# sflorescu/BWA-MEM_GPU

Measured on AMD Instinct MI355X. Metric: Mreads/s (150 bp single-end vs hg38-scale index; seed-and-extend hot path), higher is better.
Workload: dtype u16

## Files before the change

### bwa-mem_gpu_amd/bwamem_hip/lib.py

```python
from __future__ import annotations

import ctypes as C
import os

import numpy as np

_PKG = os.path.dirname(os.path.dirname(os.path.abspath(__file__)))
_u8p, _u32p, _u64p, _i32p = (C.POINTER(t) for t in (C.c_uint8, C.c_uint32, C.c_uint64, C.c_int32))


class HipLibraryMissing(RuntimeError):
    pass


def lib_path() -> str:
    return os.environ.get("BMH_LIB") or os.path.join(_PKG, "libbwamem_hip.so")


EXPORTED_SYMBOLS = [
    "bmh_last_error", "bmh_device_count", "bmh_set_device", "bmh_index_upload", "bmh_index_from_device",
    "bmh_index_free", "bmh_index_probe", "bmh_index_replicate", "bmh_rccl_where", "bmh_rccl_unique_id", "bmh_rccl_comm_init_rank", "bmh_rccl_comm_destroy", "bmh_index_broadcast_rccl", "bmh_index_replicate_all", "bmh_shard_range", "bmh_index_densify_sa", "bmh_index_build", "bmh_seed_ws_create", "bmh_seed_ws_free", "bmh_seed_batch", "bmh_seed_last_timing", "bmh_reseed_opt_default", "bmh_seed_batch_reseed", "bmh_aligner_set_reseed",
    "bmh_host_pin", "bmh_host_unpin", "bmh_extend_batch", "bmh_extend_batch_long", "bmh_extend_last_ms", "bmh_extend_last_unsupported", "bmh_extend_last_class_sizes", "bmh_extend_set_packed", "bmh_tune_set", "bmh_wtrace_start", "bmh_wtrace_stop", "bmh_wtrace_kept", "bmh_extend_release", "bmh_finalize_release", "bmh_matesw_release", "bmh_calib_gather", "bmh_calib_valu", "bmh_calib_valu_placed", "bmh_calib_last_clock",
    "bmh_jobs_frac_rep", "bmh_post_opt_default", "bmh_finalize_regs", "bmh_finalize_regs_device", "bmh_finalize_regs_device_last_ms", "bmh_sam_need_cigar", "bmh_format_sam", "bmh_free",
    "bmh_pe_opt_default", "bmh_finalize_pairs", "bmh_finalize_pairs_dev", "bmh_dedup_regs_device", "bmh_finalize_pairs_deduped", "bmh_rescue_check_counts", "bmh_sam_need_cigar_pe", "bmh_format_sam_pe",
    "bmh_chain_opt_default", "bmh_chain_last_timing", "bmh_build_jobs", "bmh_jobs_free", "bmh_jobs_sizes", "bmh_jobs_arrays", "bmh_merge_regs",
    "bmh_chain_ws_create", "bmh_chain_ws_free", "bmh_chain_set_contigs", "bmh_chain_set_alt", "bmh_effective_cpus", "bmh_aligner_create", "bmh_aligner_free", "bmh_aligner_run", "bmh_aligner_run_fasta", "bmh_chain_set_materialize", "bmh_chain_batch",
    "bmh_chain_extend", "bmh_chain_merge", "bmh_chain_extend_merge", "bmh_chain_extend_merge_timing", "bmh_cigar_batch", "bmh_cigar_release",
    "bmh_sam_select_work", "bmh_sam_select_device", "bmh_cigar_pack_work", "bmh_cigar_pack_sizes", "bmh_cigar_pack", "bmh_sam_text_work", "bmh_sam_text_sizes", "bmh_sam_text_write", "bmh_sam_text_check",
    "bwt_destroy_gpu", "bwt_restore_sa_gpu", "bwt_restore_bwt_gpu", "gpu_cpy_wrapper",
    "pre_calc_seed_intervals_wrapper", "free_gpuseed_data", "seed_gpu", "seed_gpu_last_n_reads",
    "bmh_reads_load_fasta", "bmh_reads_free", "bmh_fasta_scan",
    "bmh_reads_load", "bmh_reads_scan", "bmh_format_sam_ex", "bmh_format_sam_pe_ex", "bmh_aligner_run_file",
    "bmh_chain_ws_set_max_qlen", "bmh_aligner_set_max_qlen", "bmh_aligner_host_tail_batches",
    "bmh_index_fasta", "bmh_fasta_pack", "bmh_fasta_packed_free",
    "bmh_reads_load_files", "bmh_aligner_run_files",
    "bmh_bgzf_scan", "bmh_inflate_members_device", "bmh_inflate_members_host", "bmh_inflate_status_name", "bmh_bgzf_inflate",
# ... 460 lines not shown
    p = lib_path()
    if not os.path.exists(p):
        raise HipLibraryMissing(f"{p} not found: build it with `make -C bwa-mem_gpu_amd/csrc` "
                                "(or __graft_entry__.build()); there is no CPU fallback")
    L = C.CDLL(p)
    L.bmh_last_error.restype = C.c_char_p
    L.bmh_device_count.restype = C.c_int
    L.bmh_set_device.argtypes = [C.c_int]
    L.bmh_index_upload.restype = C.c_void_p
    L.bmh_index_upload.argtypes = [C.c_uint64, _u64p, C.c_uint64, _u32p, C.c_uint64, C.c_int, _u32p, C.c_uint64,
                                   _u32p, _u8p, C.c_uint64]
    L.bmh_index_from_device.restype = C.c_void_p
    L.bmh_index_from_device.argtypes = [C.c_uint64, _u64p, C.c_uint64, C.c_void_p, C.c_uint64, C.c_int, C.c_void_p,
                                        C.c_uint64, C.c_void_p, C.c_void_p, C.c_uint64]
    L.bmh_index_free.argtypes = [C.c_void_p]
    L.bmh_tune_set.restype = C.c_int
    L.bmh_wtrace_start.restype = C.c_int
    L.bmh_wtrace_start.argtypes = [C.c_uint32]
    L.bmh_wtrace_stop.restype = C.c_int64
    L.bmh_wtrace_stop.argtypes = [C.c_void_p, C.c_uint32]
    L.bmh_wtrace_kept.restype = C.c_uint32
    L.bmh_tune_set.argtypes = [C.c_char_p, C.c_int, C.c_int]
    L.bmh_rccl_where.restype = C.c_char_p
    L.bmh_rccl_unique_id.restype = C.c_int
    L.bmh_rccl_unique_id.argtypes = [C.c_void_p]
    L.bmh_rccl_comm_init_rank.restype = C.c_int
    L.bmh_rccl_comm_init_rank.argtypes = [C.POINTER(C.c_void_p), C.c_int, C.c_void_p, C.c_int]
    L.bmh_rccl_comm_destroy.argtypes = [C.c_void_p]
    L.bmh_index_broadcast_rccl.restype = C.c_int
    L.bmh_index_broadcast_rccl.argtypes = [C.c_void_p, C.c_int, C.c_void_p, C.POINTER(C.c_void_p), C.c_void_p]
# ... 187 lines not shown
            raise RuntimeError(f"bmh_index_densify_sa rc={rc}: " + _err(L))

    def probe(self, rows, what: str) -> np.ndarray:
        import torch
        L = load_library()
        r = torch.from_numpy(np.ascontiguousarray(rows, dtype=np.uint64).view(np.int64)).cuda()
        code = {"occ4": 0, "lf": 1, "sa": 2}[what]
        out = torch.empty(r.numel() * (4 if code == 0 else 1), dtype=torch.int64, device="cuda")
        rc = L.bmh_index_probe(self.handle, r.data_ptr(), r.numel(), code, out.data_ptr(), torch.cuda.current_stream().cuda_stream)
        if rc != 0:
            raise RuntimeError(f"bmh_index_probe rc={rc}: " + _err(L))
        torch.cuda.synchronize()
        o = out.cpu().numpy().view(np.uint64)
        return o.reshape(-1, 4) if code == 0 else o

    def free(self):
        if self.handle:
            load_library().bmh_index_free(self.handle)
            self.handle = None


class SeedWorkspace:
    def __init__(self, max_reads: int, max_bases: int, max_cands: int = 0, max_occ: int = 0):
        L = load_library()
        self.handle = L.bmh_seed_ws_create(max_reads, max_bases, max_cands, max_occ)
        if not self.handle:
            raise RuntimeError("bmh_seed_ws_create: " + _err(L))

    def seed_batch(self, index: Index, reads_t, offs_t, lens_t, min_seed_len: int = 19, stream: int = 0, reseed: "ReseedOpt | None" = None) -> SeedsT:
        L = load_library()
# ... 498 lines not shown
```

### bwa-mem_gpu_amd/csrc/bmh_internal.h

```cpp
#pragma once
#include "../../include/bwamem_hip.h"
#include "fmd_dev.h"

struct bmh_index {
	fmd_dev_t dev;
	bool owns;
	bool owns_sa;
	bool owns_blocks;
	uint64_t n_words;
};

struct bmh_ext_desc_t {
	const uint8_t *reads;
	const uint8_t *pac; long long l_pac;
	const uint32_t *jq_src;
	const uint32_t *job_side;
	uint32_t max_qlen;
	const int64_t *jt0;
	uint32_t long_cap;
};
int bmh_extend_batch_desc(const bmh_ext_desc_t *desc, const uint32_t *d_qlen, const uint32_t *d_tlen, const uint32_t *d_h0, uint32_t n,
                          const bmh_ext_params_t *p, int32_t *d_out, int32_t *d_raw, void *stream);
int bmh_extend_reserve(void *stream, uint64_t n);

#ifdef __cplusplus
// ... 97 lines not shown
```

### bwa-mem_gpu_amd/csrc/c_api.hip

```cpp
#include <hip/hip_runtime.h>
#include <stdarg.h>
#include <stdio.h>
#include <stdlib.h>
#include <string.h>
#include <map>
#include <mutex>
#include <string>
#include <vector>
#include "bmh_internal.h"

static thread_local char g_err[512] = "";

static std::mutex g_tune_mu;
static std::map<std::string, int> g_tune_set;
int bmh_tune(const char *name, int dflt)
{
	{
		std::lock_guard<std::mutex> lk(g_tune_mu);
		auto it = g_tune_set.find(name);
		if (it != g_tune_set.end()) return it->second;
	}
	const std::string env = std::string("BMH_") + name;
	const char *e = getenv(env.c_str());
	return e && *e ? atoi(e) : dflt;
// ... 146 lines not shown
	          hipMalloc((void **)&d_bits, bits_words * 4) == hipSuccess;
	if (ok && pac) ok = hipMalloc((void **)&d_pac, (size_t)(l_pac / 4 + 1) + 16) == hipSuccess && hipMemset(d_pac, 0, (size_t)(l_pac / 4 + 1) + 16) == hipSuccess;
	if (ok) ok = hipMemset(d_bwt, 0, bwt_bytes) == hipSuccess;
	if (ok) ok = hipMemcpy(d_bwt, bwt_words, (size_t)n_words * 4 < bwt_bytes ? (size_t)n_words * 4 : bwt_bytes, hipMemcpyHostToDevice) == hipSuccess;
	if (ok) ok = hipMemcpy(d_sa, sa, n_sa * 4, hipMemcpyHostToDevice) == hipSuccess;
	if (ok) ok = hipMemcpy(d_bits, sa_bits, bits_words * 4, hipMemcpyHostToDevice) == hipSuccess;
	if (ok && pac) ok = hipMemcpy(d_pac, pac, (size_t)(l_pac / 4 + 1), hipMemcpyHostToDevice) == hipSuccess;
	if (ok) ok = native_blocks(d_bwt, d_bwt, seq_len);
	if (!ok) {
		bmh_set_error("bmh_index_upload: %s", hipGetErrorString(hipGetLastError()));
		if (d_bwt) (void)hipFree(d_bwt); if (d_sa) (void)hipFree(d_sa); if (d_bits) (void)hipFree(d_bits); if (d_pac) (void)hipFree(d_pac);
		free(ix);
		return nullptr;
	}
	ix->dev.blocks = (const uint4 *)d_bwt; ix->dev.sa = d_sa; ix->dev.sa_bits = d_bits; ix->dev.pac = d_pac;
	return ix;
}

extern "C" bmh_index_t *bmh_index_from_device(uint64_t primary, const uint64_t L2[5], uint64_t seq_len, const uint32_t *d_bwt_words,
                                              uint64_t n_words, int sa_intv, const uint32_t *d_sa, uint64_t n_sa,
                                              const uint32_t *d_sa_bits, const uint8_t *d_pac, uint64_t l_pac)
{
	if (!L2 || !d_bwt_words || !d_sa || !d_sa_bits) { bmh_set_error("bmh_index_from_device: null argument"); return nullptr; }
	if (check_geometry(seq_len, L2, n_words, sa_intv, n_sa) != BMH_OK) return nullptr;
	if (((uintptr_t)d_bwt_words & 31) != 0) { bmh_set_error("bmh_index_from_device: bwt words must be 32-byte aligned"); return nullptr; }
	if (n_words < (((seq_len + 63) / 64) + 1) * 8) { bmh_set_error("bmh_index_from_device: buffer must be padded to %llu words", (unsigned long long)((((seq_len + 63) / 64) + 1) * 8)); return nullptr; }
	const size_t bwt_bytes = ((size_t)((seq_len + 63) / 64) + 1) * 32;
	void *d_native = nullptr;
	if (hipMalloc(&d_native, bwt_bytes) != hipSuccess || !native_blocks(d_bwt_words, d_native, seq_len)) {
		bmh_set_error("bmh_index_from_device: native blocks: %s", hipGetErrorString(hipGetLastError()));
		if (d_native) (void)hipFree(d_native);
		return nullptr;
	}
	bmh_index *ix = (bmh_index *)calloc(1, sizeof(bmh_index));
	ix->owns = false; ix->owns_blocks = true; ix->n_words = n_words;
	fill_dev(ix, primary, L2, seq_len, sa_intv, n_sa, d_pac ? l_pac : 0);
	ix->dev.blocks = (const uint4 *)d_native; ix->dev.sa = d_sa; ix->dev.sa_bits = d_sa_bits; ix->dev.pac = d_pac;
	return ix;
}

extern "C" int bmh_index_replicate(const bmh_index_t *src, int src_device, int dst_device, bmh_index_t **out)
{
	if (!src || !out) { bmh_set_error("bmh_index_replicate: null argument"); return BMH_EINVAL; }
	*out = nullptr;
	int prev = 0;
	if (hipGetDevice(&prev) != hipSuccess) { bmh_set_error("bmh_index_replicate: no HIP device"); return BMH_ENODEV; }
	const fmd_dev_t &f = src->dev;
	const size_t bwt_bytes = ((size_t)((f.seq_len + 63) / 64) + 1) * 32, sa_bytes = (size_t)f.n_sa * 4, bits_bytes = (size_t)(f.n_sa / 32 + 1) * 4;
	const size_t pac_bytes = f.pac ? (size_t)(f.l_pac / 4 + 1) + 16 : 0;
	bmh_index *ix = (bmh_index *)calloc(1, sizeof(bmh_index));
	*ix = *src; ix->owns = true; ix->owns_sa = false; ix->owns_blocks = false;
	void *d_bwt = nullptr, *d_sa = nullptr, *d_bits = nullptr, *d_pac = nullptr;
// ... 2 lines not shown
	if (ok && pac_bytes) ok = hipMalloc(&d_pac, pac_bytes) == hipSuccess && hipMemset(d_pac, 0, pac_bytes) == hipSuccess;
	auto cp = [&](void *dst, const void *s_, size_t n) {
		return src_device == dst_device ? hipMemcpy(dst, s_, n, hipMemcpyDeviceToDevice) == hipSuccess : hipMemcpyPeer(dst, dst_device, s_, src_device, n) == hipSuccess;
	};
	ok = ok && cp(d_bwt, f.blocks, bwt_bytes) && cp(d_sa, f.sa, sa_bytes) && cp(d_bits, f.sa_bits, bits_bytes);
	if (ok && pac_bytes) ok = cp(d_pac, f.pac, (size_t)(f.l_pac / 4 + 1));
	ok = ok && hipDeviceSynchronize() == hipSuccess;
	if (!ok) {
		bmh_set_error("bmh_index_replicate (device %d -> %d): %s", src_device, dst_device, hipGetErrorString(hipGetLastError()));
		void *ps[] = {d_bwt, d_sa, d_bits, d_pac};
		for (void *p : ps) if (p) (void)hipFree(p);
		free(ix); (void)hipSetDevice(prev);
		return BMH_ENOMEM;
	}
	ix->dev.blocks = (const uint4 *)d_bwt; ix->dev.sa = (const uint32_t *)d_sa; ix->dev.sa_bits = (const uint32_t *)d_bits; ix->dev.pac = (const uint8_t *)d_pac;
	(void)hipSetDevice(prev);
	*out = ix;
	return BMH_OK;
}

extern "C" void bmh_shard_range(uint64_t n, int rank, int world, uint32_t multiple, uint64_t *lo, uint64_t *hi)
{
	if (multiple < 1) multiple = 1;
	if (world < 1) world = 1;
	const uint64_t units = n / multiple;
	uint64_t a = units * (uint64_t)rank / (uint64_t)world * multiple, b = units * (uint64_t)(rank + 1) / (uint64_t)world * multiple;
	if (rank == world - 1) b = n;
	if (lo) *lo = a;
	if (hi) *hi = b;
}
// ... 27 lines not shown
	sa_densify_kernel<<<(unsigned)(nb < (1u << 22) ? nb : (1u << 22)), 256>>>(ix->dev, new_shift, n_new, d_sa, d_bits);
	hipError_t e = hipGetLastError();
	if (e == hipSuccess) e = hipDeviceSynchronize();
	if (e != hipSuccess) { bmh_set_error("bmh_index_densify_sa: %s", hipGetErrorString(e)); (void)hipFree(d_sa); (void)hipFree(d_bits); return BMH_ENODEV; }
	if (ix->owns || ix->owns_sa) { (void)hipFree((void *)ix->dev.sa); (void)hipFree((void *)ix->dev.sa_bits); }
	ix->dev.sa = d_sa; ix->dev.sa_bits = d_bits; ix->dev.n_sa = n_new; ix->dev.sa_shift = new_shift; ix->owns_sa = true;
	return BMH_OK;
}

extern "C" void bmh_index_free(bmh_index_t *ix)
{
	if (!ix) return;
	if (ix->owns || ix->owns_blocks) (void)hipFree((void *)ix->dev.blocks);
	if (ix->owns && ix->dev.pac) (void)hipFree((void *)ix->dev.pac);
	if (ix->owns || ix->owns_sa) { (void)hipFree((void *)ix->dev.sa); (void)hipFree((void *)ix->dev.sa_bits); }
	free(ix);
}

__global__ void __launch_bounds__(256) index_probe_kernel(fmd_dev_t f, const uint64_t *__restrict__ rows, uint64_t n, int what, uint64_t *__restrict__ out)
{
	const uint64_t t = (uint64_t)blockIdx.x * blockDim.x + threadIdx.x;
	if (t >= n) return;
	const uint64_t k = rows[t];
	if (what == 0) {
		uint64_t c4[4];
		fmd_occ4(f, k, c4);
		for (int c = 0; c < 4; ++c) out[4 * t + c] = fmd_occ1(f, k, c) == c4[c] ? c4[c] : ~0ull;
	} else if (what == 1) out[t] = fmd_inv_psi(f, k);
	else out[t] = fmd_sa(f, k);
}
// ... 12 lines not shown
```

### bwa-mem_gpu_amd/csrc/fmd_dev.h

```cpp
#pragma once
#include <hip/hip_runtime.h>
#include <stdint.h>

struct fmd_dev_t {
	uint64_t primary;
	uint64_t L2[5];
	uint64_t seq_len;
	const uint4 *blocks;
	const uint32_t *sa;
	const uint32_t *sa_bits;
	uint64_t n_sa;
	int sa_shift;
	const uint8_t *pac;
	uint64_t l_pac;
	int wave_prio;
};

__device__ __forceinline__ void fmd_wave_prio(const int p)
{
	if (p == 1) __builtin_amdgcn_s_setprio(1);
	else if (p == 2) __builtin_amdgcn_s_setprio(2);
	else if (p >= 3) __builtin_amdgcn_s_setprio(3);
}

struct blk_t { uint4 occ; uint64_t lo, hi; };

__device__ __forceinline__ uint32_t sel4(int c, uint32_t v0, uint32_t v1, uint32_t v2, uint32_t v3)
{
	const bool b0 = c & 1, b1 = c & 2;
	const uint32_t lo = b0 ? v1 : v0, hi = b0 ? v3 : v2;
	return b1 ? hi : lo;
// ... 209 lines not shown
```

### bwa-mem_gpu_amd/csrc/rccl_bcast.hip

```cpp
#include <dlfcn.h>
#include <hip/hip_runtime.h>
#include <rccl/rccl.h>
#include <stdio.h>
#include <stdlib.h>
#include <string.h>
#include <mutex>
#include <vector>
#include "bmh_internal.h"

namespace {
struct rccl_api_t {
	ncclResult_t (*GetUniqueId)(ncclUniqueId *);
	ncclResult_t (*CommInitRank)(ncclComm_t *, int, ncclUniqueId, int);
	ncclResult_t (*CommInitAll)(ncclComm_t *, int, const int *);
	ncclResult_t (*CommDestroy)(ncclComm_t);
	ncclResult_t (*CommCount)(const ncclComm_t, int *);
	ncclResult_t (*CommUserRank)(const ncclComm_t, int *);
	ncclResult_t (*Broadcast)(const void *, void *, size_t, ncclDataType_t, int, ncclComm_t, hipStream_t);
	ncclResult_t (*AllReduce)(const void *, void *, size_t, ncclDataType_t, ncclRedOp_t, ncclComm_t, hipStream_t);
	ncclResult_t (*GroupStart)();
	ncclResult_t (*GroupEnd)();
	const char *(*GetErrorString)(ncclResult_t);
	const char *where;
	bool ok;
// ... 167 lines not shown
			if (!ab.bytes[k]) continue;
			const void *sendp = is_root ? s[k] : nullptr;
			void *recvp = recv ? d[k] : (void *)s[k];
			rc = bcast_bytes(R, is_root ? sendp : recvp, recvp, k == 3 ? (size_t)(f.l_pac / 4 + 1) : ab.bytes[k], root, comm, st);
		}
		const ncclResult_t g1 = R->GroupEnd();
		if (rc == BMH_OK && g1 != ncclSuccess) { bmh_set_error("ncclGroupEnd: %s", R->GetErrorString(g1)); rc = BMH_ENODEV; }
	}
	if (rc == BMH_OK && hipStreamSynchronize(st) != hipSuccess) { bmh_set_error("bmh_index_broadcast_rccl: %s", hipGetErrorString(hipGetLastError())); rc = BMH_ENODEV; }
	if (rc != BMH_OK) { for (int k = 0; k < 4; ++k) if (d[k]) (void)hipFree(d[k]); return rc; }
	if (recv) {
		bmh_index *ix = (bmh_index *)calloc(1, sizeof(bmh_index));
		ix->dev = f; ix->owns = true; ix->n_words = h.n_words;
		ix->dev.blocks = (const uint4 *)d[0]; ix->dev.sa = (const uint32_t *)d[1]; ix->dev.sa_bits = (const uint32_t *)d[2]; ix->dev.pac = (const uint8_t *)d[3];
		if (!h.has_pac) ix->dev.l_pac = 0;
		*out = ix;
	}
	return BMH_OK;
}

extern "C" int bmh_index_replicate_all(const bmh_index_t *src, int src_device, const int *devices, int n, bmh_index_t **out, int *used_rccl)
{
	if (!src || !devices || !out || n < 1) { bmh_set_error("bmh_index_replicate_all: bad argument"); return BMH_EINVAL; }
	if (used_rccl) *used_rccl = 0;
	int prev = 0;
	HCK(hipGetDevice(&prev));
	std::vector<int> devs{src_device};
	for (int k = 0; k < n; ++k) { bool seen = false; for (int d : devs) seen = seen || d == devices[k]; if (!seen) devs.push_back(devices[k]); }
	std::vector<bmh_index_t *> per_dev(devs.size(), nullptr);
	per_dev[0] = (bmh_index_t *)src;
// ... 23 lines not shown
					for (int i = 0; i < nd && rc == BMH_OK; ++i) {
						(void)hipSetDevice(devs[i]);
						rc = bcast_bytes(R, i == 0 ? s[k] : d[i][k], i == 0 ? (void *)s[k] : d[i][k], nbytes, 0, comms[i], st[i]);
					}
				}
				const ncclResult_t g1 = R->GroupEnd();
				if (rc == BMH_OK && g1 != ncclSuccess) { bmh_set_error("ncclGroupEnd: %s", R->GetErrorString(g1)); rc = BMH_ENODEV; }
				for (int i = 0; i < nd; ++i) { (void)hipSetDevice(devs[i]); if (hipStreamSynchronize(st[i]) != hipSuccess && rc == BMH_OK) { bmh_set_error("bmh_index_replicate_all: %s", hipGetErrorString(hipGetLastError())); rc = BMH_ENODEV; } }
			}
			for (int i = 0; i < nd; ++i) { (void)hipSetDevice(devs[i]); if (st[i]) (void)hipStreamDestroy(st[i]); (void)R->CommDestroy(comms[i]); }
			if (rc == BMH_OK) {
				for (int i = 1; i < nd; ++i) {
					bmh_index *ix = (bmh_index *)calloc(1, sizeof(bmh_index));
					*ix = *src; ix->owns = true; ix->owns_sa = false; ix->owns_blocks = false;
					ix->dev.blocks = (const uint4 *)d[i][0]; ix->dev.sa = (const uint32_t *)d[i][1]; ix->dev.sa_bits = (const uint32_t *)d[i][2]; ix->dev.pac = (const uint8_t *)d[i][3];
					per_dev[i] = ix;
				}
				done = true;
				if (used_rccl) *used_rccl = 1;
			} else {
				for (int i = 1; i < nd; ++i) { (void)hipSetDevice(devs[i]); for (void *p : d[i]) if (p) (void)hipFree(p); }
			}
		}
	}
	if (!done) {
		for (int i = 1; i < nd; ++i)
			if (bmh_index_replicate(src, src_device, devs[i], &per_dev[i]) != BMH_OK) {
				for (int q = 1; q < i; ++q) { (void)hipSetDevice(devs[q]); bmh_index_free(per_dev[q]); }
				(void)hipSetDevice(prev);
				return BMH_ENOMEM;
// ... 8 lines not shown
```

### bwa-mem_gpu_amd/csrc/seed_kernels.hip

```cpp
#include <cstring>
#include <string>
#include <vector>
#include <hip/hip_runtime.h>
#include <rocprim/rocprim.hpp>
#include <stdint.h>
#include <stdio.h>
#include <stdlib.h>
#include "bmh_internal.h"
#include "wtrace.h"
#include "fmd_dev.h"
#include "seed_dev.h"


__device__ __forceinline__ int ascii_code(uint8_t ch)
{
	ch &= 0xDF;
	return ch == 'A' ? 0 : ch == 'C' ? 1 : ch == 'G' ? 2 : ch == 'T' ? 3 : 4;
}

#define PACK_READS_PER_BLOCK 64
__global__ void __launch_bounds__(256) pack_reads_kernel(const uint8_t *__restrict__ ascii, const uint32_t *__restrict__ offs,
                                                         const uint32_t *__restrict__ lens, uint32_t n_reads, uint32_t n_grp,
                                                         uint32_t lds_bytes, uint32_t *__restrict__ pk, uint32_t *__restrict__ nm)
{
// ... 73 lines not shown
                                                           unsigned long long *counter, uint64_t cap, uint32_t *__restrict__ n_cand,
                                                           unsigned long long *__restrict__ fst, const uint32_t *__restrict__ deal, uint32_t *__restrict__ iters_out)
{
	wtrace_scope_t wt_(WT_FORWARD);
	fmd_wave_prio(f.wave_prio);
	uint32_t r = blockIdx.x * blockDim.x + threadIdx.x;
	bool live = r < rv.n_reads;
	if (deal && live) r = deal[r];
	int len = live ? (int)lens[r] : 0;
	int i = 0, x = 0;
	uint32_t j = 0;
	uint64_t k = 0, l = 0, s = 0;
	enum { ST_START, ST_EXT, ST_DONE, ST_TAIL, ST_UNIQ };
	uint64_t tp = 0;
	int st = live && len > 0 ? ST_START : ST_DONE;
	cand_cursor_t cc = {0, 0};
	unsigned it_wave = 0, it_mine = 0;
	while (__any(st != ST_DONE)) {
		++it_wave; it_mine += st != ST_DONE ? 1u : 0u;
		bool want = false;
		cand_t c = {r, 0, 0, 0};
		uint64_t ck = 0;
		if (st == ST_START) {
			int b = read_base(rv, r, i);
			++i;
			if (b < 4) {
				x = i - 1;
				k = fmd_L2(f, b) + 1; s = fmd_L2(f, b + 1) - fmd_L2(f, b); l = fmd_L2(f, 3 - b) + 1;
				if (i == len) {
					want = i >= min_seed_len;
					c.xe = ((uint32_t)x << 16) | (uint32_t)i; c.j = j; c.s = (uint32_t)s; ck = k;
					st = ST_DONE;
				} else st = ST_EXT;
			} else if (i == len) st = ST_DONE;
		} else if (st == ST_EXT) {
			int b = read_base(rv, r, i);
			if (b < 4) {
				int cb = 3 - b;
				uint64_t ak[4], al[4], as[4];
				fmd_forward_ext(f, k, l, s, ak, al, as);
				const uint64_t ns = cb == 0 ? as[0] : cb == 1 ? as[1] : cb == 2 ? as[2] : as[3];
				const uint64_t nk = cb == 0 ? ak[0] : cb == 1 ? ak[1] : cb == 2 ? ak[2] : ak[3];
				const uint64_t nl = cb == 0 ? al[0] : cb == 1 ? al[1] : cb == 2 ? al[2] : al[3];
				if (ns != s) {
					want = i >= min_seed_len;
					c.xe = ((uint32_t)x << 16) | (uint32_t)i; c.j = j; c.s = (uint32_t)s; ck = k;
				}
				if (ns == 0) st = ST_START;
				else {
					k = nk; l = nl; s = ns; ++i;
					if (i == len) {
						st = ST_TAIL;
					} else if (s == 1 && f.pac) {
						tp = fmd_sa(f, k) + (uint64_t)(i - x);
						st = ST_UNIQ;
					}
				}
			} else {
				want = i >= min_seed_len;
				c.xe = ((uint32_t)x << 16) | (uint32_t)i; c.j = j; c.s = (uint32_t)s; ck = k;
				st = ST_START;
			}
		} else if (st == ST_TAIL) {
			want = i >= min_seed_len;
			c.xe = ((uint32_t)x << 16) | (uint32_t)i; c.j = j; c.s = (uint32_t)s; ck = k;
			st = ST_DONE;
		} else if (st == ST_UNIQ) {
			bool stop = false;
			for (int rep = 0; rep < FWD_UNIQ_WORDS && !stop && i < len; ++rep) {
				const int w16 = i & 15;
				const uint32_t rw = rv.pk[(size_t)(i >> 4) * rv.n_reads + r] >> (2 * w16);
				const uint32_t rm = rv.nm[(size_t)(i >> 5) * rv.n_reads + r] >> (i & 31);
				int n_av = min(16 - w16, len - i);
				const uint64_t room = tp < f.seq_len ? f.seq_len - tp : 0;
				n_av = (uint64_t)n_av < room ? n_av : (int)room;
				const uint32_t diff = rw ^ fmd_text16(f, tp);
				const uint32_t dp = (diff | (diff >> 1)) & 0x55555555u;
				const int fd = dp ? (__ffs((int)dp) - 1) >> 1 : 16;
				const int fn = (rm & 0xFFFFu) ? __ffs((int)(rm & 0xFFFFu)) - 1 : 16;
				const int m = min(min(fd, fn), n_av);
				stop = m < n_av || n_av == 0;
				i += m; tp += (uint64_t)m;
			}
			if (stop) {
				want = i >= min_seed_len;
				c.xe = ((uint32_t)x << 16) | (uint32_t)i; c.j = j; c.s = 1u; ck = k;
				st = ST_START;
			} else if (i == len) st = ST_TAIL;
		}
		if (want) ++j;
		cand_append(want, c, ck, out_a, out_k, counter, cap, cc);
	}
	cand_fill_invalid(cc, out_a, cap);
	if (live) n_cand[r] = j;
	if (iters_out && live) iters_out[r] = it_mine;
	if (fst) {
		if (live) { atomicAdd(fst + 1, (unsigned long long)it_mine); atomicAdd(fst + 8 + (it_mine / 8u < 31u ? it_mine / 8u : 31u), 1ull); }
		if ((threadIdx.x & 63) == 0) { atomicAdd(fst, (unsigned long long)it_wave); atomicAdd(fst + 2, 1ull); atomicMax(fst + 3, (unsigned long long)it_wave); atomicAdd(fst + 40 + (it_wave / 8u < 23u ? it_wave / 8u : 23u), 1ull); }
	}
}
// ... 76 lines not shown
			act = ok && i >= 0;
			if (act && (i & 15) == 15) {
				rw = rv.pk[(size_t)(i >> 4) * rv.n_reads + c.read];
				if ((i & 31) == 31) rm = rv.nm[(size_t)(i >> 5) * rv.n_reads + c.read];
			}
		}
		const unsigned long long am = __ballot(act) & above;
		const int nxt = am ? __builtin_ctzll(am) : lane;
		const uint32_t nsize = __shfl(size, nxt);
		if (act && am && nsize == size) { act = false; dropped = true; }
	}
	if (stats) {
		if (live && !RESUME) atomicAdd(stats + 8 + (st_mine < 39u ? st_mine : 39u), 1ull);
		atomicAdd(stats + 1, (unsigned long long)st_steps); atomicAdd(stats + 4, (unsigned long long)st_uniq); atomicAdd(stats + 5, (unsigned long long)st_u0); atomicAdd(stats + 6, (unsigned long long)st_x0); { const bool nowalk = !__any(live && !st_x0); if (!RESUME && lane == 0 && nowalk) atomicAdd(stats + 7, 1ull); }
		if (lane == 0) { atomicAdd(stats, (unsigned long long)st_iter); atomicAdd(stats + 2, 1ull); atomicMax(stats + 3, (unsigned long long)st_iter); }
	}
	const unsigned long long sm = __ballot(act);
	if (sm) {
		const int first = (int)__builtin_ctzll(sm);
		uint32_t base = 0;
		if (lane == first) base = atomicAdd(out_count, (uint32_t)__builtin_popcountll(sm));
		base = __shfl(base, first);
		if (act) {
			bwd_state_t s; s.lo = lo; s.hi = hi; s.read = c.read; s.t = t_out; s.x = (uint16_t)x; s.end = (uint16_t)end; s.i = (uint16_t)i; s.beg = (uint16_t)beg;
			out_state[base + (uint32_t)__builtin_popcountll(sm & ((1ull << lane) - 1ull))] = s;
		}
	}
	if (live && !act) {
		res_t o;
		o.read = c.read; o.be = ((uint32_t)beg << 16) | (uint32_t)end;
// ... 603 lines not shown
		HIPCK(rocprim::exclusive_scan(w->scan_tmp, tb, w->n_cand, w->cand_base, 0u, (size_t)n_reads + 1, rocprim::plus<uint32_t>(), st));
	}
	unsigned long long n_list = 0;
	uint32_t n_cands32 = 0;
	HIPCK(hipMemcpyAsync(&n_list, w->counter, 8, hipMemcpyDeviceToHost, st));
	HIPCK(hipMemcpyAsync(&n_cands32, w->cand_base + n_reads, 4, hipMemcpyDeviceToHost, st));
	HIPCK(hipStreamSynchronize(st));
	const unsigned long long n_cands = n_cands32;
	out->n_cands = n_cands;
	if (n_list > w->max_cands) { bmh_set_error("bmh_seed_batch: %llu candidate slots > capacity %llu", n_list, (unsigned long long)w->max_cands); return BMH_ECAPACITY; }
	if (n_list)
		cand_scatter_kernel<<<nblk(n_list, 256), 256, 0, st>>>(w->cand_a, n_list, w->cand_base, w->svals);
	{
		static const bool want_stats = getenv("BMH_SEED_STATS") != nullptr;
		unsigned long long *d_st = want_stats ? (unsigned long long *)w->counter + 8 : nullptr;
		if (want_stats) HIPCK(hipMemsetAsync(d_st, 0, 64 + 40 * 8, st));
		if (n_cands) {
			const std::vector<int> phases = [] {
				std::vector<int> v; const char *e = getenv("BMH_SEED_BWD_PHASES"); std::string t = e ? e : "";
				for (size_t p = 0; p < t.size();) { size_t q = t.find(',', p); if (q == std::string::npos) q = t.size(); const int k = atoi(t.substr(p, q - p).c_str()); if (k > 0) v.push_back(k); p = q + 1; }
				return v; }();
			const int np = (int)(phases.size() < 7 ? phases.size() : 7);
			const unsigned nb = nblk(n_cands, 256);
			const uint32_t sub_cap = ((nb + BWD_NSUB - 1) / BWD_NSUB) * 256u;
			if (np && bwd_state_reserve(w, (uint64_t)sub_cap * BWD_NSUB) != BMH_OK) return BMH_ENOMEM;
			uint32_t *cnt = w->bwd_cnt;
			if (np) HIPCK(hipMemsetAsync(cnt, 0, 4 * (size_t)np * BWD_NSUB, st));
			const int big = 0x7FFFFFFF;
			smem_backward_kernel<false><<<nb, 256, lds_pad, st>>>(f, rv, n_cands, min_seed_len, w->cand_a, w->cand_k, w->svals, w->res_a, w->res_k, d_st,
			                                                nullptr, nullptr, np ? w->bwd_state[0] : nullptr, np ? cnt : nullptr, sub_cap, np ? phases[0] : big);
			for (int ph = 1; ph <= np; ++ph)
				smem_backward_kernel<true><<<(sub_cap / 256u) * BWD_NSUB, 256, 0, st>>>(f, rv, n_cands, min_seed_len, w->cand_a, w->cand_k, w->svals, w->res_a, w->res_k, d_st,
				                                                                       w->bwd_state[(ph - 1) & 1], cnt + (size_t)(ph - 1) * BWD_NSUB, ph < np ? w->bwd_state[ph & 1] : nullptr,
				                                                                       ph < np ? cnt + (size_t)ph * BWD_NSUB : nullptr, sub_cap, ph < np ? phases[ph] : big);
		}
		if (want_stats) {
			unsigned long long h[48];
			HIPCK(hipStreamSynchronize(st));
			HIPCK(hipMemcpy(h, d_st, 64 + 40 * 8, hipMemcpyDeviceToHost));
			fprintf(stderr, "[backward] rank steps per candidate (0, 1, .. 38, 39+):");
			for (int q = 0; q < 40; ++q) fprintf(stderr, " %llu", h[8 + q]);
			fprintf(stderr, "\n");
			fprintf(stderr, "[backward] lane-steps on a one-row interval %llu (%.1f%%), candidates that start on one %llu (%.1f%%)\n", h[4], 100.0 * h[4] / (h[1] ? h[1] : 1), h[5], 100.0 * h[5] / (n_cands ? n_cands : 1));
			fprintf(stderr, "[backward] candidates of a pass that starts at read position 0 (no walk) %llu (%.1f%%); waves made of such only %llu\n", h[6], 100.0 * h[6] / (n_cands ? n_cands : 1), h[7]);
			fprintf(stderr, "[backward] candidates %llu, waves %llu (all phases), wave-iterations %llu (%.1f per wave, max %llu), lane-steps %llu (%.1f per candidate): lane utilisation %.1f%%\n",
			        (unsigned long long)n_cands, h[2], h[0], (double)h[0] / (h[2] ? h[2] : 1), h[3], h[1], (double)h[1] / (n_cands ? n_cands : 1), 100.0 * h[1] / (64.0 * (h[0] ? h[0] : 1)));
		}
	}
	HIPCK(hipEventRecord(w->ev[3], st));
	smem_filter_kernel<<<nblk(n_cands + 1, 256), 256, 0, st>>>(w->res_a, n_cands, w->occ);
	{
		size_t tb = w->scan_tmp_bytes;
		occ_keep_in fin; fin.occ = w->occ;
		HIPCK(rocprim::exclusive_scan(w->scan_tmp, tb, rocprim::make_transform_iterator(rocprim::counting_iterator<uint64_t>(0), fin), w->occ_off, (uint64_t)0,
		                              (size_t)n_cands + 1, rocprim::plus<uint64_t>(), st));
	}
	uint64_t tot[2] = {0, 0};
	HIPCK(hipMemcpyAsync(&tot[0], w->occ_off + n_cands, 8, hipMemcpyDeviceToHost, st));
	HIPCK(hipStreamSynchronize(st));
	tot[1] = tot[0] >> OCC_OFF_SHIFT; tot[0] &= OCC_OFF_MASK;
	if (n_cands >> 28) { bmh_set_error("bmh_seed_batch: more than 2^28 candidates in one batch"); return BMH_ECAPACITY; }
// ... 82 lines not shown
```

### include/bwamem_hip.h

```cpp
#ifndef BWAMEM_HIP_H
#define BWAMEM_HIP_H
#include <stddef.h>
#include <stdint.h>

#ifdef __cplusplus
extern "C" {
#endif

#define BMH_OK          0
#define BMH_ENODEV     -1
#define BMH_EINVAL     -2
#define BMH_ECAPACITY  -3
#define BMH_ENOMEM     -4

const char *bmh_last_error(void);
int bmh_device_count(void);
int bmh_set_device(int dev);


typedef struct bmh_index bmh_index_t;

bmh_index_t *bmh_index_upload(uint64_t primary, const uint64_t L2[5], uint64_t seq_len,
                              const uint32_t *bwt_words, uint64_t n_words, int sa_intv,
                              const uint32_t *sa, uint64_t n_sa, const uint32_t *sa_bits,
                              const uint8_t *pac, uint64_t l_pac);
bmh_index_t *bmh_index_from_device(uint64_t primary, const uint64_t L2[5], uint64_t seq_len,
                                   const uint32_t *d_bwt_words, uint64_t n_words, int sa_intv,
                                   const uint32_t *d_sa, uint64_t n_sa, const uint32_t *d_sa_bits,
                                   const uint8_t *d_pac, uint64_t l_pac);
void bmh_index_free(bmh_index_t *idx);
int bmh_index_probe(const bmh_index_t *idx, const uint64_t *d_rows, uint64_t n, int what, uint64_t *d_out, void *stream);

int bmh_index_replicate(const bmh_index_t *src, int src_device, int dst_device, bmh_index_t **out);

const char *bmh_rccl_where(void);
int bmh_rccl_unique_id(void *id128);
int bmh_rccl_comm_init_rank(void **comm, int nranks, const void *id128, int rank);
void bmh_rccl_comm_destroy(void *comm);
int bmh_index_broadcast_rccl(void *comm, int root, const bmh_index_t *src, bmh_index_t **out, void *stream);
int bmh_index_replicate_all(const bmh_index_t *src, int src_device, const int *devices, int n, bmh_index_t **out, int *used_rccl);
void bmh_shard_range(uint64_t n, int rank, int world, uint32_t multiple, uint64_t *lo, uint64_t *hi);

int bmh_index_densify_sa(bmh_index_t *idx, int new_intv);

#define BMH_BUILD_VERIFY 1
// ... 338 lines not shown
```

Before: 41.20.

## Add k-mer presence bitmap to prune seed candidates that cannot occur

```diff
diff --git a/bwa-mem_gpu_amd/bwamem_hip/lib.py b/bwa-mem_gpu_amd/bwamem_hip/lib.py
--- a/bwa-mem_gpu_amd/bwamem_hip/lib.py
+++ b/bwa-mem_gpu_amd/bwamem_hip/lib.py
@@ -19,7 +19,7 @@
 
 EXPORTED_SYMBOLS = [
     "bmh_last_error", "bmh_device_count", "bmh_set_device", "bmh_index_upload", "bmh_index_from_device",
-    "bmh_index_free", "bmh_index_probe", "bmh_index_replicate", "bmh_rccl_where", "bmh_rccl_unique_id", "bmh_rccl_comm_init_rank", "bmh_rccl_comm_destroy", "bmh_index_broadcast_rccl", "bmh_index_replicate_all", "bmh_shard_range", "bmh_index_densify_sa", "bmh_index_build", "bmh_seed_ws_create", "bmh_seed_ws_free", "bmh_seed_batch", "bmh_seed_last_timing", "bmh_reseed_opt_default", "bmh_seed_batch_reseed", "bmh_aligner_set_reseed",
+    "bmh_index_free", "bmh_index_kbits_info", "bmh_index_probe", "bmh_index_replicate", "bmh_rccl_where", "bmh_rccl_unique_id", "bmh_rccl_comm_init_rank", "bmh_rccl_comm_destroy", "bmh_index_broadcast_rccl", "bmh_index_replicate_all", "bmh_shard_range", "bmh_index_densify_sa", "bmh_index_build", "bmh_seed_ws_create", "bmh_seed_ws_free", "bmh_seed_batch", "bmh_seed_last_timing", "bmh_reseed_opt_default", "bmh_seed_batch_reseed", "bmh_aligner_set_reseed",
     "bmh_host_pin", "bmh_host_unpin", "bmh_extend_batch", "bmh_extend_batch_long", "bmh_extend_last_ms", "bmh_extend_last_unsupported", "bmh_extend_last_class_sizes", "bmh_extend_set_packed", "bmh_tune_set", "bmh_wtrace_start", "bmh_wtrace_stop", "bmh_wtrace_kept", "bmh_extend_release", "bmh_finalize_release", "bmh_matesw_release", "bmh_calib_gather", "bmh_calib_valu", "bmh_calib_valu_placed", "bmh_calib_last_clock",
     "bmh_jobs_frac_rep", "bmh_post_opt_default", "bmh_finalize_regs", "bmh_finalize_regs_device", "bmh_finalize_regs_device_last_ms", "bmh_sam_need_cigar", "bmh_format_sam", "bmh_free",
     "bmh_pe_opt_default", "bmh_finalize_pairs", "bmh_finalize_pairs_dev", "bmh_dedup_regs_device", "bmh_finalize_pairs_deduped", "bmh_rescue_check_counts", "bmh_sam_need_cigar_pe", "bmh_format_sam_pe",
@@ -510,6 +510,8 @@
     L.bmh_index_from_device.argtypes = [C.c_uint64, _u64p, C.c_uint64, C.c_void_p, C.c_uint64, C.c_int, C.c_void_p,
                                         C.c_uint64, C.c_void_p, C.c_void_p, C.c_uint64]
     L.bmh_index_free.argtypes = [C.c_void_p]
+    L.bmh_index_kbits_info.restype = C.c_int
+    L.bmh_index_kbits_info.argtypes = [C.c_void_p, C.POINTER(C.c_int), C.POINTER(C.c_void_p), _u64p]
     L.bmh_tune_set.restype = C.c_int
     L.bmh_wtrace_start.restype = C.c_int
     L.bmh_wtrace_start.argtypes = [C.c_uint32]
@@ -727,6 +729,23 @@
         o = out.cpu().numpy().view(np.uint64)
         return o.reshape(-1, 4) if code == 0 else o
 
+    def kbits_info(self) -> tuple:
+        L = load_library()
+        k, p, n = C.c_int(0), C.c_void_p(None), C.c_uint64(0)
+        rc = L.bmh_index_kbits_info(self.handle, C.byref(k), C.byref(p), C.byref(n))
+        if rc != 0:
+            raise RuntimeError(f"bmh_index_kbits_info rc={rc}: " + _err(L))
+        return int(k.value), int(p.value or 0), int(n.value)
+
+    def kbits_to_host(self) -> np.ndarray:
+        import torch
+        _, p, n = self.kbits_info()
+        if not n:
+            return np.zeros(0, np.uint32)
+        buf = torch.empty(n, dtype=torch.int32, device="cuda")
+        _memcpy_d2d(buf.data_ptr(), p, n * 4)
+        return buf.cpu().numpy().view(np.uint32)
+
     def free(self):
         if self.handle:
             load_library().bmh_index_free(self.handle)
diff --git a/bwa-mem_gpu_amd/csrc/bmh_internal.h b/bwa-mem_gpu_amd/csrc/bmh_internal.h
--- a/bwa-mem_gpu_amd/csrc/bmh_internal.h
+++ b/bwa-mem_gpu_amd/csrc/bmh_internal.h
@@ -9,6 +9,8 @@
 	bool owns_blocks;
 	uint64_t n_words;
 };
+void bmh_kbits_attach(bmh_index *ix);
+void bmh_kbits_free(bmh_index *ix);
 
 struct bmh_ext_desc_t {
 	const uint8_t *reads;
diff --git a/bwa-mem_gpu_amd/csrc/c_api.hip b/bwa-mem_gpu_amd/csrc/c_api.hip
--- a/bwa-mem_gpu_amd/csrc/c_api.hip
+++ b/bwa-mem_gpu_amd/csrc/c_api.hip
@@ -184,6 +184,7 @@
 		return nullptr;
 	}
 	ix->dev.blocks = (const uint4 *)d_bwt; ix->dev.sa = d_sa; ix->dev.sa_bits = d_bits; ix->dev.pac = d_pac;
+	bmh_kbits_attach(ix);
 	return ix;
 }
 
@@ -206,6 +207,7 @@
 	ix->owns = false; ix->owns_blocks = true; ix->n_words = n_words;
 	fill_dev(ix, primary, L2, seq_len, sa_intv, n_sa, d_pac ? l_pac : 0);
 	ix->dev.blocks = (const uint4 *)d_native; ix->dev.sa = d_sa; ix->dev.sa_bits = d_sa_bits; ix->dev.pac = d_pac;
+	bmh_kbits_attach(ix);
 	return ix;
 }
 
@@ -238,6 +240,7 @@
 		return BMH_ENOMEM;
 	}
 	ix->dev.blocks = (const uint4 *)d_bwt; ix->dev.sa = (const uint32_t *)d_sa; ix->dev.sa_bits = (const uint32_t *)d_bits; ix->dev.pac = (const uint8_t *)d_pac;
+	bmh_kbits_attach(ix);
 	(void)hipSetDevice(prev);
 	*out = ix;
 	return BMH_OK;
@@ -295,6 +298,7 @@
 	if (ix->owns || ix->owns_blocks) (void)hipFree((void *)ix->dev.blocks);
 	if (ix->owns && ix->dev.pac) (void)hipFree((void *)ix->dev.pac);
 	if (ix->owns || ix->owns_sa) { (void)hipFree((void *)ix->dev.sa); (void)hipFree((void *)ix->dev.sa_bits); }
+	bmh_kbits_free(ix);
 	free(ix);
 }
 
diff --git a/bwa-mem_gpu_amd/csrc/fmd_dev.h b/bwa-mem_gpu_amd/csrc/fmd_dev.h
--- a/bwa-mem_gpu_amd/csrc/fmd_dev.h
+++ b/bwa-mem_gpu_amd/csrc/fmd_dev.h
@@ -14,7 +14,18 @@
 	const uint8_t *pac;
 	uint64_t l_pac;
 	int wave_prio;
+	const uint32_t *kbits;
+	int kbits_k;
 };
+
+__host__ __device__ __forceinline__ uint64_t kbits_mask(int K) { return (1ull << (2 * K)) - 1ull; }
+__host__ __device__ __forceinline__ uint64_t kbits_n_words(int K) { return K >= 3 ? 1ull << (2 * K - 5) : 1ull; }
+__host__ __device__ __forceinline__ void kbits_slot(uint64_t key, uint64_t &word, uint32_t &bit) { word = key >> 5; bit = 1u << (uint32_t)(key & 31); }
+__device__ __forceinline__ uint64_t kbits_push(uint64_t win, uint32_t syms, int n, int K)
+{
+	const uint64_t v = (uint64_t)syms & ((1ull << (2 * n)) - 1ull);
+	return n >= K ? v >> (2 * (n - K)) : (win >> (2 * n)) | (v << (2 * (K - n)));
+}
 
 __device__ __forceinline__ void fmd_wave_prio(const int p)
 {
diff --git a/bwa-mem_gpu_amd/csrc/kmer_bits.hip b/bwa-mem_gpu_amd/csrc/kmer_bits.hip
--- /dev/null
+++ b/bwa-mem_gpu_amd/csrc/kmer_bits.hip
@@ -0,0 +1,82 @@
+#include <hip/hip_runtime.h>
+#include <stdint.h>
+#include <stdio.h>
+#include <stdlib.h>
+#include "bmh_internal.h"
+
+#define KBITS_MAX_K 18
+#define KBITS_PER_THREAD 8
+
+extern "C" int bmh_kbits_k_for(uint64_t seq_len)
+{
+	int K = 1;
+	while (K < KBITS_MAX_K && ((1ull << (2 * K)) >> 3) < seq_len) ++K;
+	return K;
+}
+
+__global__ void __launch_bounds__(256) kbits_build_kernel(fmd_dev_t f, int K, uint64_t n_win, uint32_t *__restrict__ bits)
+{
+	const uint64_t n_grp = (n_win + KBITS_PER_THREAD - 1) / KBITS_PER_THREAD, mask = kbits_mask(K);
+	for (uint64_t g = (uint64_t)blockIdx.x * blockDim.x + threadIdx.x; g < n_grp; g += (uint64_t)gridDim.x * blockDim.x) {
+		const uint64_t t0 = g * KBITS_PER_THREAD;
+		const uint64_t w = (uint64_t)fmd_text16(f, t0) | ((uint64_t)fmd_text16(f, t0 + 16) << 32);
+#pragma unroll
+		for (int p = 0; p < KBITS_PER_THREAD; ++p) {
+			if (t0 + (uint64_t)p >= n_win) break;
+			uint64_t word; uint32_t bit;
+			kbits_slot((w >> (2 * p)) & mask, word, bit);
+			atomicOr(&bits[word], bit);
+		}
+	}
+}
+
+void bmh_kbits_attach(bmh_index *ix)
+{
+	ix->dev.kbits = nullptr; ix->dev.kbits_k = 0;
+	const fmd_dev_t &f = ix->dev;
+	const char *sw = getenv("BMH_SEED_KBITS");
+	if (sw && sw[0] == '0') return;
+	if (!f.pac || f.l_pac == 0 || f.seq_len != 2 * f.l_pac) return;
+	const int K = bmh_kbits_k_for(f.seq_len);
+	if (f.seq_len < (uint64_t)K) return;
+	const uint64_t n_words = kbits_n_words(K), n_win = f.seq_len - (uint64_t)K + 1;
+	uint32_t *d = nullptr;
+	hipEvent_t e0 = nullptr, e1 = nullptr;
+	bool ok = hipMalloc((void **)&d, (size_t)n_words * 4) == hipSuccess;
+	ok = ok && hipEventCreate(&e0) == hipSuccess && hipEventCreate(&e1) == hipSuccess;
+	ok = ok && hipEventRecord(e0, 0) == hipSuccess && hipMemsetAsync(d, 0, (size_t)n_words * 4, 0) == hipSuccess;
+	if (ok) {
+		const uint64_t nb = ((n_win + KBITS_PER_THREAD - 1) / KBITS_PER_THREAD + 255) / 256;
+		kbits_build_kernel<<<(unsigned)(nb < (1u << 20) ? nb : (1u << 20)), 256>>>(f, K, n_win, d);
+		ok = hipGetLastError() == hipSuccess && hipEventRecord(e1, 0) == hipSuccess && hipDeviceSynchronize() == hipSuccess;
+	}
+	if (ok && getenv("BMH_SEED_STATS")) {
+		float ms = 0.f;
+		(void)hipEventElapsedTime(&ms, e0, e1);
+		fprintf(stderr, "[kbits] K = %d, %llu windows, bitmap %.3f MiB, built in %.1f ms\n", K, (unsigned long long)n_win, (double)n_words * 4.0 / 1048576.0, ms);
+	}
+	if (e0) (void)hipEventDestroy(e0);
+	if (e1) (void)hipEventDestroy(e1);
+	if (!ok) {
+		(void)hipGetLastError();
+		if (d) (void)hipFree(d);
+		return;
+	}
+	ix->dev.kbits = d; ix->dev.kbits_k = K;
+}
+
+void bmh_kbits_free(bmh_index *ix)
+{
+	if (ix->dev.kbits) (void)hipFree((void *)ix->dev.kbits);
+	ix->dev.kbits = nullptr; ix->dev.kbits_k = 0;
+}
+
+extern "C" int bmh_index_kbits_info(const bmh_index_t *ix, int *k, const uint32_t **d_bits, uint64_t *n_words)
+{
+	if (!ix) { bmh_set_error("bmh_index_kbits_info: null index"); return BMH_EINVAL; }
+	const bool has = ix->dev.kbits != nullptr;
+	if (k) *k = has ? ix->dev.kbits_k : 0;
+	if (d_bits) *d_bits = ix->dev.kbits;
+	if (n_words) *n_words = has ? kbits_n_words(ix->dev.kbits_k) : 0;
+	return BMH_OK;
+}
diff --git a/bwa-mem_gpu_amd/csrc/rccl_bcast.hip b/bwa-mem_gpu_amd/csrc/rccl_bcast.hip
--- a/bwa-mem_gpu_amd/csrc/rccl_bcast.hip
+++ b/bwa-mem_gpu_amd/csrc/rccl_bcast.hip
@@ -205,6 +205,7 @@
 		ix->dev = f; ix->owns = true; ix->n_words = h.n_words;
 		ix->dev.blocks = (const uint4 *)d[0]; ix->dev.sa = (const uint32_t *)d[1]; ix->dev.sa_bits = (const uint32_t *)d[2]; ix->dev.pac = (const uint8_t *)d[3];
 		if (!h.has_pac) ix->dev.l_pac = 0;
+		bmh_kbits_attach(ix);
 		*out = ix;
 	}
 	return BMH_OK;
@@ -258,6 +259,8 @@
 					bmh_index *ix = (bmh_index *)calloc(1, sizeof(bmh_index));
 					*ix = *src; ix->owns = true; ix->owns_sa = false; ix->owns_blocks = false;
 					ix->dev.blocks = (const uint4 *)d[i][0]; ix->dev.sa = (const uint32_t *)d[i][1]; ix->dev.sa_bits = (const uint32_t *)d[i][2]; ix->dev.pac = (const uint8_t *)d[i][3];
+					(void)hipSetDevice(devs[i]);
+					bmh_kbits_attach(ix);
 					per_dev[i] = ix;
 				}
 				done = true;
diff --git a/bwa-mem_gpu_amd/csrc/seed_kernels.hip b/bwa-mem_gpu_amd/csrc/seed_kernels.hip
--- a/bwa-mem_gpu_amd/csrc/seed_kernels.hip
+++ b/bwa-mem_gpu_amd/csrc/seed_kernels.hip
@@ -111,6 +111,9 @@
 	enum { ST_START, ST_EXT, ST_DONE, ST_TAIL, ST_UNIQ };
 	uint64_t tp = 0;
 	int st = live && len > 0 ? ST_START : ST_DONE;
+	const int kK = (f.kbits && min_seed_len >= f.kbits_k) ? f.kbits_k : 0;
+	uint64_t win = 0;
+	int clean = 0;
 	cand_cursor_t cc = {0, 0};
 	unsigned it_wave = 0, it_mine = 0;
 	while (__any(st != ST_DONE)) {
@@ -118,14 +121,23 @@
 		bool want = false;
 		cand_t c = {r, 0, 0, 0};
 		uint64_t ck = 0;
+		const bool kprobe = kK && (st == ST_EXT || st == ST_TAIL) && i >= min_seed_len && i - x < kK;
+		uint32_t kw = 0, kb = 0;
+		if (kprobe && clean >= kK) { uint64_t wd; kbits_slot(win, wd, kb); kw = f.kbits[wd]; }
+		const bool kdead = kprobe && !(kw & kb);
 		if (st == ST_START) {
 			int b = read_base(rv, r, i);
 			++i;
+			win = kbits_push(win, (uint32_t)b & 3u, 1, kK); clean = b < 4 ? min(clean + 1, 255) : 0;
 			if (b < 4) {
 				x = i - 1;
 				k = fmd_L2(f, b) + 1; s = fmd_L2(f, b + 1) - fmd_L2(f, b); l = fmd_L2(f, 3 - b) + 1;
 				if (i == len) {
 					want = i >= min_seed_len;
+					if (want && kK > 1) {
+						uint64_t wd; uint32_t bt; kbits_slot(win, wd, bt);
+						want = clean >= kK && (f.kbits[wd] & bt);
+					}
 					c.xe = ((uint32_t)x << 16) | (uint32_t)i; c.j = j; c.s = (uint32_t)s; ck = k;
 					st = ST_DONE;
 				} else st = ST_EXT;
@@ -140,12 +152,13 @@
 				const uint64_t nk = cb == 0 ? ak[0] : cb == 1 ? ak[1] : cb == 2 ? ak[2] : ak[3];
 				const uint64_t nl = cb == 0 ? al[0] : cb == 1 ? al[1] : cb == 2 ? al[2] : al[3];
 				if (ns != s) {
-					want = i >= min_seed_len;
+					want = i >= min_seed_len && !kdead;
 					c.xe = ((uint32_t)x << 16) | (uint32_t)i; c.j = j; c.s = (uint32_t)s; ck = k;
 				}
 				if (ns == 0) st = ST_START;
 				else {
 					k = nk; l = nl; s = ns; ++i;
+					win = kbits_push(win, (uint32_t)b, 1, kK); clean = min(clean + 1, 255);
 					if (i == len) {
 						st = ST_TAIL;
 					} else if (s == 1 && f.pac) {
@@ -154,12 +167,12 @@
 					}
 				}
 			} else {
-				want = i >= min_seed_len;
+				want = i >= min_seed_len && !kdead;
 				c.xe = ((uint32_t)x << 16) | (uint32_t)i; c.j = j; c.s = (uint32_t)s; ck = k;
 				st = ST_START;
 			}
 		} else if (st == ST_TAIL) {
-			want = i >= min_seed_len;
+			want = i >= min_seed_len && !kdead;
 			c.xe = ((uint32_t)x << 16) | (uint32_t)i; c.j = j; c.s = (uint32_t)s; ck = k;
 			st = ST_DONE;
 		} else if (st == ST_UNIQ) {
@@ -178,9 +191,14 @@
 				const int m = min(min(fd, fn), n_av);
 				stop = m < n_av || n_av == 0;
 				i += m; tp += (uint64_t)m;
+				win = kbits_push(win, rw, m, kK); clean = min(clean + m, 255);
 			}
 			if (stop) {
 				want = i >= min_seed_len;
+				if (want && i - x < kK) {
+					uint64_t wd; uint32_t bt; kbits_slot(win, wd, bt);
+					want = clean >= kK && (f.kbits[wd] & bt);
+				}
 				c.xe = ((uint32_t)x << 16) | (uint32_t)i; c.j = j; c.s = 1u; ck = k;
 				st = ST_START;
 			} else if (i == len) st = ST_TAIL;
@@ -287,6 +305,7 @@
 		if (live && !RESUME) atomicAdd(stats + 8 + (st_mine < 39u ? st_mine : 39u), 1ull);
 		atomicAdd(stats + 1, (unsigned long long)st_steps); atomicAdd(stats + 4, (unsigned long long)st_uniq); atomicAdd(stats + 5, (unsigned long long)st_u0); atomicAdd(stats + 6, (unsigned long long)st_x0); { const bool nowalk = !__any(live && !st_x0); if (!RESUME && lane == 0 && nowalk) atomicAdd(stats + 7, 1ull); }
 		if (lane == 0) { atomicAdd(stats, (unsigned long long)st_iter); atomicAdd(stats + 2, 1ull); atomicMax(stats + 3, (unsigned long long)st_iter); }
+		if (live && !act && end - beg < min_seed_len) { atomicAdd(stats + 48, (unsigned long long)st_mine); atomicAdd(stats + 49, 1ull); if (!dropped) { atomicAdd(stats + 50, (unsigned long long)st_mine); atomicAdd(stats + 51, 1ull); } }
 	}
 	const unsigned long long sm = __ballot(act);
 	if (sm) {
@@ -920,7 +939,7 @@
 	{
 		static const bool want_stats = getenv("BMH_SEED_STATS") != nullptr;
 		unsigned long long *d_st = want_stats ? (unsigned long long *)w->counter + 8 : nullptr;
-		if (want_stats) HIPCK(hipMemsetAsync(d_st, 0, 64 + 40 * 8, st));
+		if (want_stats) HIPCK(hipMemsetAsync(d_st, 0, 52 * 8, st));
 		if (n_cands) {
 			const std::vector<int> phases = [] {
 				std::vector<int> v; const char *e = getenv("BMH_SEED_BWD_PHASES"); std::string t = e ? e : "";
@@ -941,9 +960,9 @@
 				                                                                       ph < np ? cnt + (size_t)ph * BWD_NSUB : nullptr, sub_cap, ph < np ? phases[ph] : big);
 		}
 		if (want_stats) {
-			unsigned long long h[48];
+			unsigned long long h[52];
 			HIPCK(hipStreamSynchronize(st));
-			HIPCK(hipMemcpy(h, d_st, 64 + 40 * 8, hipMemcpyDeviceToHost));
+			HIPCK(hipMemcpy(h, d_st, sizeof(h), hipMemcpyDeviceToHost));
 			fprintf(stderr, "[backward] rank steps per candidate (0, 1, .. 38, 39+):");
 			for (int q = 0; q < 40; ++q) fprintf(stderr, " %llu", h[8 + q]);
 			fprintf(stderr, "\n");
@@ -951,6 +970,9 @@
 			fprintf(stderr, "[backward] candidates of a pass that starts at read position 0 (no walk) %llu (%.1f%%); waves made of such only %llu\n", h[6], 100.0 * h[6] / (n_cands ? n_cands : 1), h[7]);
 			fprintf(stderr, "[backward] candidates %llu, waves %llu (all phases), wave-iterations %llu (%.1f per wave, max %llu), lane-steps %llu (%.1f per candidate): lane utilisation %.1f%%\n",
 			        (unsigned long long)n_cands, h[2], h[0], (double)h[0] / (h[2] ? h[2] : 1), h[3], h[1], (double)h[1] / (n_cands ? n_cands : 1), 100.0 * h[1] / (64.0 * (h[0] ? h[0] : 1)));
+			fprintf(stderr, "[backward] candidates that end shorter than min_seed_len %llu (%.1f%%) with %llu lane-steps (%.1f%% of all); of these not dropped in lockstep %llu with %llu lane-steps (%.1f%%); K-mer bitmap %s (%.1f candidates per read)\n",
+			        h[49], 100.0 * h[49] / (n_cands ? n_cands : 1), h[48], 100.0 * h[48] / (h[1] ? h[1] : 1), h[51], h[50], 100.0 * h[50] / (h[1] ? h[1] : 1),
+			        (f.kbits && min_seed_len >= f.kbits_k) ? "on" : "off", (double)n_cands / n_reads);
 		}
 	}
 	HIPCK(hipEventRecord(w->ev[3], st));
diff --git a/include/bwamem_hip.h b/include/bwamem_hip.h
--- a/include/bwamem_hip.h
+++ b/include/bwamem_hip.h
@@ -29,6 +29,7 @@
                                    const uint32_t *d_sa, uint64_t n_sa, const uint32_t *d_sa_bits,
                                    const uint8_t *d_pac, uint64_t l_pac);
 void bmh_index_free(bmh_index_t *idx);
+int bmh_index_kbits_info(const bmh_index_t *idx, int *k, const uint32_t **d_bits, uint64_t *n_words);
 int bmh_index_probe(const bmh_index_t *idx, const uint64_t *d_rows, uint64_t n, int what, uint64_t *d_out, void *stream);
 
 int bmh_index_replicate(const bmh_index_t *src, int src_device, int dst_device, bmh_index_t **out);
```

Result: faster. 44.75 (median of 6 runs) (+8.6%).
